# gradslam/gradslam

Hardware: NVIDIA H100
Metric: PointFusion frames/sec (640x480, B=8) (higher is better)
Workload: dtype f32

## Files before the change

gradslam_b200/_C.py:

```python
import ctypes
import os

import torch

_HERE = os.path.dirname(os.path.abspath(__file__))
LIB_PATH = os.environ.get("GSX_LIB_PATH") or os.path.join(_HERE, "_lib", "libgsx.so")

c_f32p = ctypes.c_void_p
c_i32p = ctypes.c_void_p
c_i64 = ctypes.c_int64
c_int = ctypes.c_int
c_float = ctypes.c_float
c_double = ctypes.c_double
c_u32 = ctypes.c_uint32
c_vp = ctypes.c_void_p

SIGNATURES = {
    "gsx_version": (c_int, []),
    "gsx_last_error": (ctypes.c_char_p, []),
    "gsx_backproject_normals_fwd": (
        c_int, [c_vp, c_i64, c_vp, c_i64, c_vp, c_i64, c_int, c_int, c_int, c_int, c_vp, c_vp, c_vp, c_vp, c_vp]),
    "gsx_backproject_normals_bwd_scratch_bytes": (c_i64, [c_int, c_int, c_int, c_int]),
    "gsx_backproject_normals_bwd": (
        c_int, [c_vp, c_i64, c_vp, c_i64, c_vp, c_i64, c_int, c_int, c_int, c_int, c_vp, c_vp, c_vp, c_vp, c_vp, c_vp,
                c_vp, c_i64, c_vp]),
    "gsx_fusion_workspace_bytes": (c_i64, [c_int, c_int, c_int]),
    "gsx_fusion_workspace_stats_offset": (c_i64, [c_int, c_int, c_int]),
    "gsx_fusion_frame_records": (
        c_int, [c_vp, c_i64, c_vp, c_i64, c_vp, c_i64, c_vp, c_vp, c_vp, c_int, c_int, c_int, c_double, c_vp, c_vp]),
    "gsx_fusion_project_select": (
        c_int, [c_vp, c_vp, c_i64, c_i64, c_vp, c_i64, c_vp, c_i64, c_int, c_int, c_int, c_float, c_float, c_vp, c_vp]),
    "gsx_fusion_merge_append": (
        c_int, [c_vp, c_vp, c_int, c_vp, c_vp, c_i64, c_vp, c_i64, c_int, c_int, c_int, c_vp, c_vp, c_vp, c_vp]),
    "gsx_fusion_merge_append_bwd": (
        c_int, [c_vp, c_vp, c_vp, c_vp, c_int, c_i64, c_vp, c_vp, c_i64, c_vp, c_vp, c_vp, c_vp, c_int, c_int, c_int,
                c_double, c_vp, c_vp, c_vp, c_vp, c_vp, c_vp, c_vp]),
    "gsx_pointfusion_sequence_groups": (c_int, [c_int]),
    "gsx_pointfusion_sequence_workspace_bytes": (c_i64, [c_int, c_int, c_int]),
    "gsx_pointfusion_sequence_gt": (
        c_int, [c_vp, c_vp, c_vp, c_i64, c_i64, c_vp, c_vp, c_vp, c_vp, c_int, c_int, c_int, c_int, c_int, c_int,
                c_float, c_float, c_double, c_vp, c_vp, c_vp]),
    "gsx_fusion_prune_scratch_bytes": (c_i64, [c_int, c_i64]),
    "gsx_fusion_prune_unstable": (
        c_int, [c_vp, c_vp, c_vp, c_i64, c_vp, c_int, c_int, c_int, c_float, c_int, c_vp, c_vp, c_i64, c_vp]),
    "gsx_fusion_prune_unstable_bwd": (c_int, [c_vp, c_vp, c_i64, c_vp, c_vp, c_i64, c_int, c_vp, c_vp, c_vp]),
    "gsx_pointfusion_sequence_gt_prune": (
        c_int, [c_vp, c_vp, c_vp, c_i64, c_i64, c_vp, c_vp, c_vp, c_vp, c_int, c_int, c_int, c_int, c_int, c_int,
                c_float, c_float, c_double, c_vp, c_vp, c_int, c_float, c_vp, c_i64, c_vp, c_vp]),
    "gsx_debug_fail_at_frame": (None, [c_int]),
    "gsx_debug_set_k2_grid_cap": (None, [c_int]),
    "gsx_peer_export": (c_int, [c_vp, c_vp, c_vp, c_vp]),
    "gsx_peer_open": (c_int, [c_vp, c_i64, c_vp]),
    "gsx_peer_close_all": (c_int, []),
    "gsx_peer_copy_rows": (c_int, [c_vp, c_i64, c_vp, c_i64, c_i64, c_i64, c_vp]),
    "gsx_ingest_raw": (c_int, [c_vp, c_vp, c_i64, c_double, c_int, c_vp, c_vp, c_vp]),
    "gsx_ingest_calibration": (c_int, [c_vp, c_i64, c_int, c_double, c_double, c_vp, c_vp, c_int, c_int, c_vp, c_vp,
                                       c_vp]),
    "gsx_compact_scratch_bytes": (c_i64, [c_i64]),
    "gsx_compact_indices": (c_int, [c_vp, c_i64, c_vp, c_vp, c_vp, c_u32, c_vp]),
    "gsx_active_eval": (c_int, [c_vp, c_vp, c_i64, c_i64, c_vp, c_i64, c_vp, c_i64, c_int, c_int, c_int, c_vp, c_vp,
                                c_vp]),
    "gsx_similar_eval": (c_int, [c_vp, c_i64, c_vp, c_i64, c_vp, c_vp, c_int, c_int, c_int, c_float, c_float, c_vp,
                                 c_vp]),
    "gsx_unique_select": (c_int, [c_vp, c_i64, c_vp, c_i64, c_vp, c_int, c_int, c_int, c_vp, c_vp, c_vp, c_vp]),
    "gsx_records_from_table": (c_int, [c_vp, c_i64, c_i64, c_int, c_int, c_int, c_vp, c_vp]),
    "gsx_knn1_scratch_bytes": (c_i64, [c_int, c_int, c_int]),
    "gsx_icp_tgt_scratch_bytes": (c_i64, [c_int, c_i64]),
    "gsx_knn1": (c_int, [c_vp, c_vp, c_int, c_vp, c_vp, c_int, c_int, c_vp, c_vp, c_vp, c_i64, c_int, c_vp]),
    "gsx_icp_normal_eq_scratch_bytes": (c_i64, [c_int]),
    "gsx_icp_normal_eq_fwd": (c_int, [c_vp, c_int, c_vp, c_vp, c_vp, c_vp, c_vp, c_i64, c_vp]),
    "gsx_icp_normal_eq_bwd": (c_int, [c_vp, c_int, c_vp, c_vp, c_vp, c_vp, c_vp, c_vp, c_vp, c_vp]),
    "gsx_icp_normal_eq_batched_fwd": (c_int, [c_vp, c_vp, c_int, c_vp, c_vp, c_int, c_int, c_vp, c_vp, c_vp, c_i64, c_vp]),
    "gsx_icp_normal_eq_batched_bwd": (c_int, [c_vp, c_vp, c_int, c_vp, c_vp, c_int, c_int, c_vp, c_vp, c_vp, c_vp, c_vp,
                                              c_vp]),
    "gsx_icp_solve_fwd": (c_int, [c_vp, c_vp, c_int, c_vp, c_vp, c_vp]),
    "gsx_icp_solve_bwd": (c_int, [c_vp, c_vp, c_int, c_vp, c_vp, c_vp, c_vp, c_vp]),
    "gsx_icp_update_fwd": (c_int, [c_vp, c_vp, c_vp, c_vp, c_vp, c_int, c_int, c_float, c_float, c_float, c_float,
                                   c_vp, c_vp, c_vp, c_vp]),
    "gsx_icp_update_bwd": (c_int, [c_vp, c_vp, c_vp, c_vp, c_vp, c_int, c_int, c_float, c_float, c_float, c_float,
                                   c_vp, c_vp, c_vp, c_vp, c_vp, c_vp, c_vp, c_vp, c_vp]),
    "gsx_rigid_transform_fwd": (c_int, [c_vp, c_i64, c_vp, c_vp, c_vp]),
    "gsx_rigid_transform_bwd_scratch_bytes": (c_i64, [c_i64]),
    "gsx_rigid_transform_batched_fwd": (c_int, [c_vp, c_vp, c_i64, c_int, c_vp, c_vp, c_vp]),
    "gsx_rigid_transform_batched_bwd": (c_int, [c_vp, c_vp, c_i64, c_int, c_vp, c_vp, c_vp, c_vp, c_vp, c_i64, c_vp]),
    "gsx_rigid_transform_bwd": (c_int, [c_vp, c_i64, c_vp, c_vp, c_vp, c_vp, c_vp, c_i64, c_vp]),
    "gsx_icp_align_scratch_bytes": (c_i64, [c_int, c_int, c_int]),
    "gsx_icp_align": (
        c_int, [c_vp, c_vp, c_int, c_vp, c_vp, c_vp, c_int, c_int, c_vp, c_int, c_int, c_float, c_int, c_float,
                c_float, c_float, c_float, c_float, c_vp, c_vp, c_vp, c_i64, c_vp]),
    "gsx_icp_workspace_bytes": (c_i64, [c_int, c_int, c_int, c_int, c_i64]),
    "gsx_icp_localize": (
        c_int, [c_vp, c_vp, c_i64, c_i64, c_vp, c_i64, c_vp, c_i64, c_vp, c_i64, c_int, c_int, c_int, c_int,
                c_int, c_int, c_float, c_int, c_float, c_float, c_float, c_float, c_float, c_vp, c_i64, c_vp, c_i64,
                c_vp, c_i64, c_u32, c_vp, c_vp]),
    "gsx_icp_projective_workspace_bytes": (c_i64, [c_int, c_int, c_int, c_int]),
    "gsx_icp_localize_projective": (
        c_int, [c_vp, c_vp, c_i64, c_i64, c_vp, c_i64, c_vp, c_i64, c_vp, c_i64, c_int, c_int, c_int, c_int, c_int,
                c_int, c_float, c_int, c_float, c_float, c_float, c_float, c_float, c_vp, c_i64, c_vp, c_i64, c_vp]),
    "gsx_icp_project_associate": (
        c_int, [c_vp, c_vp, c_int, c_vp, c_vp, c_vp, c_i64, c_vp, c_i64, c_int, c_int, c_int, c_int, c_float, c_vp, c_vp,
                c_vp]),
    "gsx_render_views": (
        c_int, [c_vp, c_vp, c_vp, c_i64, c_i64, c_vp, c_i64, c_vp, c_i64, c_int, c_int, c_int, c_int, c_vp, c_vp, c_vp,
                c_vp, c_vp, c_vp]),
    "gsx_render_views_bwd_scratch_bytes": (c_i64, [c_int, c_int, c_int, c_int]),
    "gsx_render_views_bwd": (
        c_int, [c_vp, c_vp, c_i64, c_vp, c_i64, c_vp, c_i64, c_vp, c_int, c_int, c_int, c_int, c_vp, c_vp, c_vp, c_vp,
                c_vp, c_vp, c_vp, c_vp, c_i64, c_vp]),
}

_lib = None


def lib():
    global _lib
    if _lib is None:
        if not os.path.exists(LIB_PATH):
            raise RuntimeError(
                "gradslam_b200: CUDA extension %s is missing. Build it with `python __graft_entry__.py build`. "
                "There is no CPU fallback." % LIB_PATH
            )
        handle = ctypes.CDLL(LIB_PATH)
        for name, (res, args) in SIGNATURES.items():
            fn = getattr(handle, name)
            fn.restype = res
            fn.argtypes = args
        _lib = handle
    return _lib


def check(rc, what):
    if rc != 0:
        raise RuntimeError("%s failed (status %d): %s" % (what, rc, lib().gsx_last_error().decode()))
# ... 45 lines not shown
```

gradslam_b200/csrc/gsx_fusion.cu:

```cuda
#include "gsx_common.cuh"
#include "gsx_exp.cuh"
#include "gsx_fusion_ws.cuh"
#include "gsx_thresholds.h"
#include "../../include/gsx.h"

namespace gsx {

constexpr int kBlock = 256;

__device__ __forceinline__ float confidence_exp(float sq_norm, float two_sigma_sq) {
  const float x = (-sq_norm) / two_sigma_sq;
  if (!(x >= -17.0f)) return 0.0f;
  return exp_f32_via_f64(x);
}
__device__ __forceinline__ float confidence_alpha(float sq_norm, float two_sigma_sq) {
  return fminf(fmaxf(confidence_exp(sq_norm, two_sigma_sq), 1e-7f), 1.01f);
}

struct FrameRecArgs {
  const float *depth;
  int64_t depth_bstride;
  const float *K;
  int64_t K_bstride;
  const float *poses;
  int64_t pose_bstride;
  const float *gv, *gn, *vloc;
  int B, H, W;
  float two_sigma_sq;
  Workspace ws;
};

constexpr int kRecTW = 32, kRecTH = 8;

__device__ __forceinline__ void store_frame_header(const FrameRecArgs &a, int b) {
  FrameHeader hd = {};
  hd.from_maps = a.gv != nullptr;
  if (!hd.from_maps) {
    hd.cam.k = load_kinv(a.K + b * a.K_bstride);
    if (a.poses) hd.cam.pose = load_rigid(a.poses + b * a.pose_bstride);
    hd.cam.posed = a.poses != nullptr;
  }
  hd.two_sigma_sq = a.two_sigma_sq;
  hd.depth = a.depth + b * a.depth_bstride;
  a.ws.hdr[b] = hd;
}

template <bool kAlpha>
__device__ __forceinline__ void frame_values(const FrameHeader &hd, bool from_maps, const Rigid *pose,
                                             const float4 *nrec, const float4 *vrec, int h, int w, int H, int W, float dc,
                                             float3 &gn, float4 &fv) {
  if (from_maps) {
    const float4 n = __ldg(nrec + h * W + w);
    gn = make_float3(n.x, n.y, n.z);
    fv = __ldg(vrec + h * W + w);
    return;
  }
  const FrameSample f = frame_sample_from(load_stencil_around(hd.depth, dc, h, w, H, W), hd.cam.k, pose, h, w, H, W);
  gn = f.gn;
  fv = make_float4(f.gv.x, f.gv.y, f.gv.z,
                   kAlpha ? confidence_alpha((f.v.x * f.v.x + f.v.y * f.v.y) + f.v.z * f.v.z, hd.two_sigma_sq) : 0.0f);
}

__device__ __forceinline__ float frame_depth(const FrameHeader &hd, bool from_maps, const float4 *nrec, int pix) {
  return from_maps ? __ldg(nrec + pix).w : __ldg(hd.depth + pix);
}

__device__ __forceinline__ void load_frame_header(FrameHeader &s, const FrameHeader *g) {
  constexpr int kWords = (int)(sizeof(FrameHeader) / 4);
  const int i = (int)threadIdx.x - 64;
  if (i >= 0 && i < kWords) reinterpret_cast<int *>(&s)[i] = __ldg(reinterpret_cast<const int *>(g) + i);
}

template <bool kFromMaps>
__global__ void __launch_bounds__(kRecTW *kRecTH) k_frame_records(FrameRecArgs a) {
  const int b = blockIdx.z;
  const int tid = threadIdx.y * kRecTW + threadIdx.x;
  const int lin = (blockIdx.y * gridDim.x + blockIdx.x) * (kRecTW * kRecTH) + tid;
  if (lin < a.ws.tiles) a.ws.tile_state[(int64_t)b * a.ws.tiles + lin] = 0ull;
  if (lin == 0) {
    a.ws.ticket[b] = 0u;
    store_frame_header(a, b);
  }
  const int w = blockIdx.x * kRecTW + threadIdx.x, h = blockIdx.y * kRecTH + threadIdx.y;
  if (w >= a.W || h >= a.H) return;
  const int P = a.H * a.W;
  const int pix = h * a.W + w;
  const int64_t i = (int64_t)b * P + pix;
  if (kFromMaps) {
    const int64_t o = i * 3;
    const float vx = __ldg(a.vloc + o), vy = __ldg(a.vloc + o + 1), vz = __ldg(a.vloc + o + 2);
    a.ws.nrec[i] = make_float4(__ldg(a.gn + o), __ldg(a.gn + o + 1), __ldg(a.gn + o + 2),
                               __ldg(a.depth + b * a.depth_bstride + pix));
    a.ws.vrec[i] = make_float4(__ldg(a.gv + o), __ldg(a.gv + o + 1), __ldg(a.gv + o + 2),
                               confidence_alpha((vx * vx + vy * vy) + vz * vz, a.two_sigma_sq));
  }
  a.ws.win[i] = 0u;
}

int launch_frame_records(const FrameRecArgs &a, cudaStream_t stream) {
  if (a.B == 0) return 0;
  const dim3 grid((unsigned)((a.W + kRecTW - 1) / kRecTW), (unsigned)((a.H + kRecTH - 1) / kRecTH), (unsigned)a.B);
  const dim3 block(kRecTW, kRecTH);
  if (a.gv)
    k_frame_records<true><<<grid, block, 0, stream>>>(a);
  else
    k_frame_records<false><<<grid, block, 0, stream>>>(a);
  GSX_CHECK_LAUNCH("gsx_fusion_frame_records");
  return 0;
}

struct ProjectArgs {
  const float *geo;
  const int32_t *counts;
  int64_t cap;
  const float *poses;
  int64_t pose_bstride;
  const float *K;
  int64_t K_bstride;
  int B;
  ImageBounds ib;
  float dot_th;
  float d2_max;
  const float4 *nrec, *vrec;
  const FrameHeader *hdr;
  unsigned int *win;
  unsigned long long *stats;
};

#ifndef GSX_K2_MINB
#define GSX_K2_MINB 4
#endif

struct MapRow {
  float4 a, b;
};
__device__ __forceinline__ MapRow load_map_row(const float *geo, int64_t n) {
  MapRow m;
  m.a = __ldg(reinterpret_cast<const float4 *>(geo + n * kGeoW));
  m.b = __ldg(reinterpret_cast<const float4 *>(geo + n * kGeoW + 4));
  return m;
}

template <bool kFromMaps>
__device__ __forceinline__ void select_rows(const ProjectArgs &a, const LiveCamera &s_cam, const FrameHeader &s_hdr,
                                            unsigned int *s_act, int b, int count) {
  const int P = a.ib.H * a.ib.W;
  const float *geo = a.geo + (int64_t)b * a.cap * kGeoW;
  const float4 *nrec = a.nrec + (int64_t)b * P, *vrec = a.vrec + (int64_t)b * P;
  unsigned int *win = a.win + (int64_t)b * P;
  const int64_t stride = (int64_t)gridDim.x * kBlock;
  int64_t n = (int64_t)blockIdx.x * kBlock + threadIdx.x;
  int pend_pix = -1;
  unsigned int pend_n = 0u, pend_old = 0u;
  unsigned long long pend_key = 0ull;
  float3 pend_fv = make_float3(0.f, 0.f, 0.f);
  MapRow cur = load_map_row(geo, n < count ? n : 0);
  for (; n < count; n += stride) {
    const MapRow m = cur;
    const int64_t nn = n + stride;
    if (nn < count) cur = load_map_row(geo, nn);
    const PixelHit hit = project(s_cam, a.ib, m.a.x, m.a.y, m.a.z);
    if (hit.in_frustum) {
      {
        const unsigned int am = __activemask();
        if ((int)(threadIdx.x & 31) == __ffs(am) - 1) atomicAdd(s_act + (threadIdx.x >> 5), (unsigned int)__popc(am));
      }
      const int pix = hit.h * a.ib.W + hit.w;
      float3 gn;
      float4 fv;
      frame_values<false>(s_hdr, kFromMaps, s_hdr.cam.posed ? &s_hdr.cam.pose : nullptr, nrec, vrec, hit.h, hit.w,
                          a.ib.H, a.ib.W, frame_depth(s_hdr, kFromMaps, nrec, pix), gn, fv);
      const float dot = (gn.x * m.a.w + gn.y * m.b.x) + gn.z * m.b.y;
      const float3 fv3 = make_float3(fv.x, fv.y, fv.z);
      const float d2 = ray_d2(fv3, m.a.x, m.a.y, m.a.z);
      const bool live = (d2 <= a.d2_max) && (dot > a.dot_th);
      if (pend_pix >= 0) {
        argmin_settle(win + pend_pix, pend_n, pend_key, pend_fv, geo, pend_old);
        pend_pix = -1;
      }
      if (live) {
        pend_n = (unsigned int)n;
        pend_key = argmin_key_hi(m.b.z, d2);
        pend_fv = fv3;
        pend_old = argmin_claim(win + pix, pend_n);
        pend_pix = pix;
      }
    }
  }
  if (pend_pix >= 0) argmin_settle(win + pend_pix, pend_n, pend_key, pend_fv, geo, pend_old);
}

__global__ void __launch_bounds__(kBlock, GSX_K2_MINB) k_project_select(ProjectArgs a) {
  __shared__ LiveCamera s_cam;
  __shared__ FrameHeader s_hdr;
  __shared__ unsigned int s_act[kBlock / 32];
  const int b = blockIdx.y;
  const int count = a.counts[b];
  if ((int64_t)blockIdx.x * kBlock >= count) return;
  load_live_camera(s_cam, a.poses, a.pose_bstride, a.K, a.K_bstride, b);
  load_frame_header(s_hdr, a.hdr + b);
  if (threadIdx.x < kBlock / 32) s_act[threadIdx.x] = 0u;
  __syncthreads();
  if (s_hdr.from_maps)
    select_rows<true>(a, s_cam, s_hdr, s_act, b, count);
  else
    select_rows<false>(a, s_cam, s_hdr, s_act, b, count);
  __syncthreads();
  if (threadIdx.x == 0) {
    unsigned int t = 0;
#pragma unroll
    for (int i = 0; i < kBlock / 32; ++i) t += s_act[i];
    if (t) atomicAdd(a.stats + 2 * b, (unsigned long long)t);
  }
}

#ifndef GSX_K2_CTAS_PER_SM
#define GSX_K2_CTAS_PER_SM 24
#endif

static int g_k2_grid_cap = 0;

int launch_project_select(const ProjectArgs &a, int64_t max_count, cudaStream_t stream) {
  if (a.B == 0 || max_count <= 0) return 0;
  int64_t bx = (max_count + kBlock - 1) / kBlock;
  const int64_t cap_blocks = g_k2_grid_cap > 0 ? (int64_t)g_k2_grid_cap : (int64_t)kNumSMs * GSX_K2_CTAS_PER_SM;
  if (bx * a.B > cap_blocks) bx = (cap_blocks + a.B - 1) / a.B;
  if (bx < 1) bx = 1;
  k_project_select<<<dim3((unsigned)bx, (unsigned)a.B), kBlock, 0, stream>>>(a);
  GSX_CHECK_LAUNCH("gsx_fusion_project_select");
  return 0;
}

struct MergeArgs {
  float *geo, *col;
  int with_cc;
  const int32_t *counts_in;
  int32_t *counts_out;
  int64_t cap;
  const float *rgb;
  int64_t rgb_bstride;
  int B, H, W;
  Workspace ws;
  int32_t *overflow;
  int32_t *assoc;
};

constexpr unsigned int kMergeEpoch = 1u;

#ifndef GSX_K4_MINB
#define GSX_K4_MINB 4
#endif

__device__ __forceinline__ void prefetch_l2(const float *p) { asm volatile("prefetch.global.L2 [%0];" ::"l"(p)); }

template <bool kAssoc>
__global__ void __launch_bounds__(kMB, GSX_K4_MINB) k_merge_append(MergeArgs a) {
  __shared__ int s_tile;
  __shared__ int s_warp_sums[kPix][kMB / 32];
  __shared__ int s_matched[kMB / 32];
  __shared__ int s_excl;
  __shared__ __align__(16) float s_rgb[kTilePix * 3];
  __shared__ FrameHeader s_hdr;
  const int b = blockIdx.x % a.B;
  const int T = a.ws.tiles;
  if (threadIdx.x == 0) s_tile = (int)atomicAdd(a.ws.ticket + b, 1u);
  load_frame_header(s_hdr, a.ws.hdr + b);
  const int count_in = a.counts_in[b];
  __syncthreads();
  const int tile = s_tile;
  const int P = a.H * a.W;
  const int lane = threadIdx.x & 31, warp = threadIdx.x >> 5;
  const int pix0 = tile * kTilePix;
  const unsigned int *win = a.ws.win + (int64_t)b * P;
  const float4 *nrec = a.ws.nrec + (int64_t)b * P, *vrec = a.ws.vrec + (int64_t)b * P;
  const float *rgb = a.rgb + b * a.rgb_bstride + (int64_t)pix0 * 3;

  const int tile_px = min(kTilePix, P - pix0);
  if ((reinterpret_cast<uintptr_t>(rgb) & 15) == 0) {
    const int n4 = (tile_px * 3) >> 2;
    for (int i = threadIdx.x; i < n4; i += kMB)
      reinterpret_cast<float4 *>(s_rgb)[i] = __ldg(reinterpret_cast<const float4 *>(rgb) + i);
    for (int i = (n4 << 2) + threadIdx.x; i < tile_px * 3; i += kMB) s_rgb[i] = __ldg(rgb + i);
  } else {
    for (int i = threadIdx.x; i < tile_px * 3; i += kMB) s_rgb[i] = __ldg(rgb + i);
  }

  int pix[kPix];
  unsigned int slot[kPix];
  float dep[kPix];
  bool matched[kPix], is_new[kPix];
#pragma unroll
  for (int j = 0; j < kPix; ++j) {
    pix[j] = pix0 + j * kMB + threadIdx.x;
    slot[j] = 0u;
    dep[j] = 0.0f;
    if (pix[j] < P) {
      slot[j] = win[pix[j]];
      dep[j] = frame_depth(s_hdr, s_hdr.from_maps, nrec, pix[j]);
    }
    matched[j] = a.with_cc && slot[j] != 0u;
    if (matched[j]) {
      const int64_t n = (int64_t)slot[j] - 1;
      prefetch_l2(a.geo + ((int64_t)b * a.cap + n) * kGeoW);
      prefetch_l2(a.col + ((int64_t)b * a.cap + n) * kColW);
    }
  }
  int n_matched = 0;
#pragma unroll
  for (int j = 0; j < kPix; ++j) n_matched += matched[j] ? 1 : 0;
  n_matched = __reduce_add_sync(0xffffffffu, n_matched);
  if (lane == 0) s_matched[warp] = n_matched;
  int new_off[kPix];
  const int block_total = block_offsets<kMB, kPix>(
      [&](int j) {
        is_new[j] = (pix[j] < P) && (dep[j] > 0.0f) && !matched[j];
        return is_new[j];
      },
      new_off, s_warp_sums,
      [&] {
        if (threadIdx.x == 0) {
          int t = 0;
#pragma unroll
          for (int i = 0; i < kMB / 32; ++i) t += s_matched[i];
          if (t) atomicAdd(a.ws.stats + 2 * b + 1, (unsigned long long)t);
        }
      });
  unsigned long long *state = a.ws.tile_state + (int64_t)b * T;
  if (threadIdx.x == 0) publish_tile(state, tile, T, kMergeEpoch, kTileAggregate, (unsigned)block_total);

  float *geo = a.geo + (int64_t)b * a.cap * kGeoW;
  float *col = a.col + (int64_t)b * a.cap * kColW;

  float4 fv[kPix];
  float3 fn[kPix];
#pragma unroll
  for (int j = 0; j < kPix; ++j) {
    if (matched[j] || is_new[j]) {
      const int ph = pix[j] / a.W;
      frame_values<true>(s_hdr, s_hdr.from_maps, s_hdr.cam.posed ? &s_hdr.cam.pose : nullptr, nrec, vrec, ph, pix[j] - ph * a.W, a.H, a.W, dep[j], fn[j], fv[j]);
    }
  }

  float4 g0[kPix], g1[kPix], c4[kPix];
#pragma unroll
  for (int j = 0; j < kPix; ++j) {
    if (matched[j]) {
      const int64_t n = (int64_t)slot[j] - 1;
      g0[j] = *reinterpret_cast<const float4 *>(geo + n * kGeoW);
      g1[j] = *reinterpret_cast<const float4 *>(geo + n * kGeoW + 4);
      c4[j] = *reinterpret_cast<const float4 *>(col + n * kColW);
    }
  }
#pragma unroll
  for (int j = 0; j < kPix; ++j) {
    if (matched[j]) {
      const int64_t n = (int64_t)slot[j] - 1;
      const float alpha = fv[j].w;
      const float c0 = g1[j].z;
      const float tot = c0 + alpha;
      const float inv = 1.0f / ((tot == 0.0f) ? 1.0f : tot);
      const float *fc = s_rgb + (j * kMB + (int)threadIdx.x) * 3;
      float4 o0, o1, oc;
      o0.x = ((c0 * g0[j].x) + (alpha * fv[j].x)) * inv;
      o0.y = ((c0 * g0[j].y) + (alpha * fv[j].y)) * inv;
      o0.z = ((c0 * g0[j].z) + (alpha * fv[j].z)) * inv;
      o0.w = ((c0 * g0[j].w) + (alpha * fn[j].x)) * inv;
      o1.x = ((c0 * g1[j].x) + (alpha * fn[j].y)) * inv;
      o1.y = ((c0 * g1[j].y) + (alpha * fn[j].z)) * inv;
      o1.z = tot;
      o1.w = 0.0f;
      oc.x = ((c0 * c4[j].x) + (alpha * fc[0])) * inv;
      oc.y = ((c0 * c4[j].y) + (alpha * fc[1])) * inv;
      oc.z = ((c0 * c4[j].z) + (alpha * fc[2])) * inv;
      oc.w = 0.0f;
      *reinterpret_cast<float4 *>(geo + n * kGeoW) = o0;
      *reinterpret_cast<float4 *>(geo + n * kGeoW + 4) = o1;
      *reinterpret_cast<float4 *>(col + n * kColW) = oc;
      if (kAssoc) a.assoc[(int64_t)b * P + pix[j]] = -(int32_t)(n + 1);
    }
  }

  if (warp == 0) {
    const unsigned int excl = lookback_warp(state, tile, T, kMergeEpoch, (unsigned)block_total);
    if (lane == 0) s_excl = (int)excl;
  }
  __syncthreads();
  const int64_t base = (int64_t)count_in + s_excl;
#pragma unroll
  for (int j = 0; j < kPix; ++j) {
    if (is_new[j]) {
      const int64_t n = base + new_off[j];
      if (n < a.cap) {
        const float *fc = s_rgb + (j * kMB + (int)threadIdx.x) * 3;
        *reinterpret_cast<float4 *>(geo + n * kGeoW) = make_float4(fv[j].x, fv[j].y, fv[j].z, fn[j].x);
        *reinterpret_cast<float4 *>(geo + n * kGeoW + 4) =
            make_float4(fn[j].y, fn[j].z, a.with_cc ? fv[j].w : 0.0f, 0.0f);
        *reinterpret_cast<float4 *>(col + n * kColW) = make_float4(fc[0], fc[1], fc[2], 0.0f);
        if (kAssoc) a.assoc[(int64_t)b * P + pix[j]] = (int32_t)(n + 1);
      } else {
        *a.overflow = 1;
      }
    }
  }
  if (tile == T - 1 && threadIdx.x == 0) {
    const int64_t total = base + block_total;
    a.counts_out[b] = (int32_t)(total < a.cap ? total : a.cap);
  }
}

int launch_merge_append(const MergeArgs &a, cudaStream_t stream) {
  if (a.B == 0) return 0;
  const dim3 grid((unsigned)(a.ws.tiles * a.B));
  if (a.assoc)
    k_merge_append<true><<<grid, kMB, 0, stream>>>(a);
  else
    k_merge_append<false><<<grid, kMB, 0, stream>>>(a);
  GSX_CHECK_LAUNCH("gsx_fusion_merge_append");
  return 0;
}

struct MergeBwdArgs {
  const int32_t *assoc;
  const int32_t *counts_in;
  const float *geo, *col;
  int with_cc;
  int64_t cap_in;
  const float *g_geo, *g_col;
  int64_t cap_out;
  const float *gv, *gn, *rgb, *vloc;
  float *d_geo, *d_col;
  float *d_gv, *d_gn, *d_rgb, *d_vloc;
  int B, P;
  float two_sigma_sq;
};

__global__ void __launch_bounds__(256) k_merge_bwd_rows(MergeBwdArgs a) {
  const int b = blockIdx.y;
  const int64_t n = (int64_t)blockIdx.x * blockDim.x + threadIdx.x;
  if (n >= a.cap_in) return;
  const bool live = n < a.counts_in[b] && n < a.cap_out;
  const int64_t ri = (int64_t)b * a.cap_in + n, ro = (int64_t)b * a.cap_out + n;
  float4 z = make_float4(0.f, 0.f, 0.f, 0.f), g0 = z, g1 = z, gc = z;
  if (live && a.g_geo) {
    g0 = *reinterpret_cast<const float4 *>(a.g_geo + ro * kGeoW);
    g1 = *reinterpret_cast<const float4 *>(a.g_geo + ro * kGeoW + 4);
    g1.w = 0.0f;
    if (!a.with_cc) g1.z = 0.0f;
  }
  if (live && a.g_col) {
    gc = *reinterpret_cast<const float4 *>(a.g_col + ro * kColW);
    gc.w = 0.0f;
  }
  *reinterpret_cast<float4 *>(a.d_geo + ri * kGeoW) = g0;
  *reinterpret_cast<float4 *>(a.d_geo + ri * kGeoW + 4) = g1;
  *reinterpret_cast<float4 *>(a.d_col + ri * kColW) = gc;
}

__global__ void __launch_bounds__(256) k_merge_bwd_pixels(MergeBwdArgs a) {
  const int b = blockIdx.y;
  const int pix = blockIdx.x * blockDim.x + threadIdx.x;
  if (pix >= a.P) return;
  const int64_t fi = ((int64_t)b * a.P + pix) * 3;
  const int32_t as = a.assoc[(int64_t)b * a.P + pix];
  float dgv[3] = {0.f, 0.f, 0.f}, dgn[3] = {0.f, 0.f, 0.f}, dc[3] = {0.f, 0.f, 0.f}, dv[3] = {0.f, 0.f, 0.f};
  if (as != 0) {
    const int64_t n = (as > 0) ? (int64_t)as - 1 : -(int64_t)as - 1;
    const int64_t ro = (int64_t)b * a.cap_out + n;
    float g[9];
#pragma unroll
    for (int q = 0; q < 6; ++q) g[q] = a.g_geo ? a.g_geo[ro * kGeoW + q] : 0.0f;
#pragma unroll
    for (int q = 0; q < 3; ++q) g[6 + q] = a.g_col ? a.g_col[ro * kColW + q] : 0.0f;
    const float gcc = (a.g_geo && a.with_cc) ? a.g_geo[ro * kGeoW + 6] : 0.0f;
    const float vx = a.vloc[fi], vy = a.vloc[fi + 1], vz = a.vloc[fi + 2];
    const float sq = (vx * vx + vy * vy) + vz * vz;
    const float e = (float)exp((double)((-sq) / a.two_sigma_sq));
    float d_alpha = gcc;
    if (as > 0) {
#pragma unroll
      for (int q = 0; q < 3; ++q) {
        dgv[q] = g[q];
        dgn[q] = g[3 + q];
        dc[q] = g[6 + q];
      }
    } else {
      const int64_t ri = (int64_t)b * a.cap_in + n;
      const float alpha = fminf(fmaxf(e, 1e-7f), 1.01f);
      const float c0 = a.geo[ri * kGeoW + 6];
      const float tot = c0 + alpha;
      const bool degenerate = tot == 0.0f;
      const float inv = 1.0f / (degenerate ? 1.0f : tot);
      const float dinv = degenerate ? 0.0f : -(inv * inv);
      float f[9], m[9];
#pragma unroll
      for (int q = 0; q < 3; ++q) {
        f[q] = a.gv[fi + q];
        f[3 + q] = a.gn[fi + q];
        f[6 + q] = a.rgb[fi + q];
        m[q] = a.geo[ri * kGeoW + q];
        m[3 + q] = a.geo[ri * kGeoW + 3 + q];
        m[6 + q] = a.col[ri * kColW + q];
      }
      float d_c0 = gcc;
      float dm[9], df[9];
#pragma unroll
      for (int q = 0; q < 9; ++q) {
        const float num = c0 * m[q] + alpha * f[q];
        dm[q] = g[q] * c0 * inv;
        df[q] = g[q] * alpha * inv;
        d_c0 += g[q] * (m[q] * inv + num * dinv);
        d_alpha += g[q] * (f[q] * inv + num * dinv);
      }
#pragma unroll
      for (int q = 0; q < 6; ++q) a.d_geo[ri * kGeoW + q] = dm[q];
      a.d_geo[ri * kGeoW + 6] = d_c0;
#pragma unroll
      for (int q = 0; q < 3; ++q) {
        a.d_col[ri * kColW + q] = dm[6 + q];
        dgv[q] = df[q];
        dgn[q] = df[3 + q];
        dc[q] = df[6 + q];
      }
    }
    if (e >= 1e-7f && e <= 1.01f) {
      const float s = d_alpha * e * (-2.0f / a.two_sigma_sq);
      dv[0] = s * vx;
      dv[1] = s * vy;
      dv[2] = s * vz;
    }
  }
#pragma unroll
  for (int q = 0; q < 3; ++q) {
    a.d_gv[fi + q] = dgv[q];
    a.d_gn[fi + q] = dgn[q];
    a.d_rgb[fi + q] = dc[q];
    a.d_vloc[fi + q] = dv[q];
  }
}

static Workspace group_workspace(void *workspace, int B_total, int b0, int H, int W) {
  const int64_t P = (int64_t)H * W;
  Workspace ws = fusion_workspace(workspace, B_total, H, W);
  ws.nrec += (int64_t)b0 * P;
  ws.vrec += (int64_t)b0 * P;
  ws.hdr += b0;
  ws.win += (int64_t)b0 * P;
  ws.tile_state += (int64_t)b0 * ws.tiles;
  ws.ticket += b0;
  ws.stats += 2 * b0;
  return ws;
}

int fusion_records_group(const float *poses, int64_t pose_bs, const float *K, int64_t K_bs, const float *depth,
                         int64_t d_bs, int B_total, int b0, int nb, int H, int W, double sigma, void *workspace,
                         cudaStream_t st) {
  FrameRecArgs fa{depth + (int64_t)b0 * d_bs, d_bs, K + (int64_t)b0 * K_bs, K_bs, poses + (int64_t)b0 * pose_bs, pose_bs,
                  nullptr, nullptr, nullptr, nb, H, W, (float)(2.0 * (sigma * sigma)),
                  group_workspace(workspace, B_total, b0, H, W)};
  return launch_frame_records(fa, st);
}

int fusion_update_group(float *geo, float *col, const int32_t *cin, int32_t *cout, int64_t cap, int64_t max_count,
                        const float *poses, int64_t pose_bs, const float *K, int64_t K_bs, const float *rgb,
                        int64_t rgb_bs, int B_total, int b0, int nb, int H, int W, float dist_th, float dot_th,
                        void *workspace, int32_t *overflow, cudaStream_t st) {
  const Workspace ws = group_workspace(workspace, B_total, b0, H, W);
  float *ggeo = geo + (int64_t)b0 * cap * kGeoW, *gcol = col + (int64_t)b0 * cap * kColW;
  if (max_count > 0) {
    ProjectArgs pa{ggeo, cin + b0, cap, poses + (int64_t)b0 * pose_bs, pose_bs, K + (int64_t)b0 * K_bs, K_bs, nb,
                   image_bounds(H, W), dot_th, sqrt_lt_threshold(dist_th), ws.nrec, ws.vrec, ws.hdr, ws.win, ws.stats};
    const int rc = launch_project_select(pa, max_count, st);
    if (rc) return rc;
  }
  MergeArgs ma{ggeo, gcol, 1, cin + b0, cout + b0, cap, rgb + (int64_t)b0 * rgb_bs, rgb_bs, nb, H, W, ws, overflow, nullptr};
  return launch_merge_append(ma, st);
}

int64_t fusion_workspace_bytes(int B, int H, int W) {
  int64_t bytes;
  fusion_workspace(nullptr, B, H, W, &bytes);
  return bytes;
}

}

using namespace gsx;

extern "C" int64_t gsx_fusion_workspace_bytes(int B, int H, int W) {
  if (B < 0 || H < 0 || W < 0) return -1;
  return fusion_workspace_bytes(B, H, W);
}

extern "C" int64_t gsx_fusion_workspace_stats_offset(int B, int H, int W) {
  if (B < 0 || H < 0 || W < 0) return -1;
  return (int64_t)reinterpret_cast<uintptr_t>(fusion_workspace(nullptr, B, H, W).stats);
}

static bool aligned16(const void *p) { return (reinterpret_cast<uintptr_t>(p) & 15) == 0; }

extern "C" int gsx_fusion_frame_records(const float *depth, int64_t depth_bstride, const float *intrinsics,
                                        int64_t K_bstride, const float *poses, int64_t pose_bstride,
                                        const float *gvertex, const float *gnormal, const float *vertex, int B, int H,
                                        int W, double sigma, void *workspace, void *stream) {
  GSX_CHECK_ARG(B >= 0 && H >= 2 && W >= 2, "gsx_fusion_frame_records: bad extents B=%d H=%d W=%d", B, H, W);
  if (B == 0) return 0;
  GSX_CHECK_ARG(depth && workspace, "gsx_fusion_frame_records: null pointer");
  GSX_CHECK_ARG((gvertex && gnormal && vertex) || (!gvertex && !gnormal && !vertex && intrinsics),
                "gsx_fusion_frame_records: pass the three frame maps, or none of them together with the intrinsics");
  GSX_CHECK_ARG(aligned16(workspace), "gsx_fusion_frame_records: the workspace must be 16-byte aligned");
  FrameRecArgs a{depth, depth_bstride, intrinsics, K_bstride, poses, pose_bstride, gvertex, gnormal, vertex, B, H, W,
                 (float)(2.0 * (sigma * sigma)), fusion_workspace(workspace, B, H, W)};
  return launch_frame_records(a, (cudaStream_t)stream);
}

extern "C" int gsx_fusion_project_select(const float *map_geometry, const int32_t *counts, int64_t capacity,
                                         int64_t max_count, const float *poses, int64_t pose_bstride,
                                         const float *intrinsics, int64_t K_bstride, int B, int H, int W,
                                         float dist_th, float dot_th, void *workspace, void *stream) {
  GSX_CHECK_ARG(B >= 0 && H >= 2 && W >= 2, "gsx_fusion_project_select: bad extents B=%d H=%d W=%d", B, H, W);
  if (max_count <= 0 || B == 0) return 0;
  GSX_CHECK_ARG(map_geometry && counts, "gsx_fusion_project_select: null map pointer");
  GSX_CHECK_ARG(poses && intrinsics && workspace, "gsx_fusion_project_select: null frame pointer");
  GSX_CHECK_ARG(aligned16(map_geometry) && aligned16(workspace),
                "gsx_fusion_project_select: geometry rows and workspace must be 16-byte aligned");
  GSX_CHECK_ARG(max_count <= capacity, "gsx_fusion_project_select: max_count %lld > capacity %lld",
                (long long)max_count, (long long)capacity);
  const Workspace ws = fusion_workspace(workspace, B, H, W);
  ProjectArgs a{map_geometry, counts, capacity, poses, pose_bstride, intrinsics, K_bstride, B, image_bounds(H, W),
                dot_th, sqrt_lt_threshold(dist_th), ws.nrec, ws.vrec, ws.hdr, ws.win, ws.stats};
  return launch_project_select(a, max_count, (cudaStream_t)stream);
}

extern "C" void gsx_debug_set_k2_grid_cap(int ctas) { g_k2_grid_cap = ctas > 0 ? ctas : 0; }

extern "C" int gsx_fusion_merge_append(float *map_geometry, float *map_colors, int with_ccounts,
                                       const int32_t *counts_in, int32_t *counts_out, int64_t capacity,
                                       const float *rgb, int64_t rgb_bstride, int B, int H, int W, void *workspace,
                                       int32_t *overflow_flag, int32_t *assoc_out, void *stream) {
  GSX_CHECK_ARG(B >= 0 && H >= 2 && W >= 2, "gsx_fusion_merge_append: bad extents B=%d H=%d W=%d", B, H, W);
  if (B == 0) return 0;
  GSX_CHECK_ARG(map_geometry && map_colors && counts_in && counts_out, "gsx_fusion_merge_append: null map pointer");
  GSX_CHECK_ARG(counts_in != counts_out, "gsx_fusion_merge_append: counts_in and counts_out must not alias");
  GSX_CHECK_ARG(rgb && workspace && overflow_flag, "gsx_fusion_merge_append: null frame pointer");
  GSX_CHECK_ARG(aligned16(map_geometry) && aligned16(map_colors) && aligned16(workspace),
                "gsx_fusion_merge_append: map rows and workspace must be 16-byte aligned");
  GSX_CHECK_ARG(capacity <= 0x7fffffffll, "gsx_fusion_merge_append: capacity must fit int32 (counts are int32)");
  MergeArgs a{map_geometry, map_colors, with_ccounts ? 1 : 0, counts_in, counts_out, capacity, rgb, rgb_bstride, B, H,
              W, fusion_workspace(workspace, B, H, W), overflow_flag, assoc_out};
  return launch_merge_append(a, (cudaStream_t)stream);
}

extern "C" int gsx_fusion_merge_append_bwd(const int32_t *assoc, const int32_t *counts_in, const float *map_geometry,
                                           const float *map_colors, int with_ccounts, int64_t capacity_in,
                                           const float *g_geometry, const float *g_colors, int64_t capacity_out,
                                           const float *gvertex, const float *gnormal, const float *rgb,
                                           const float *vertex, int B, int H, int W, double sigma,
                                           float *d_map_geometry, float *d_map_colors, float *d_gvertex,
                                           float *d_gnormal, float *d_rgb, float *d_vertex, void *stream) {
  GSX_CHECK_ARG(B >= 0 && H >= 2 && W >= 2, "gsx_fusion_merge_append_bwd: bad extents B=%d H=%d W=%d", B, H, W);
  if (B == 0) return 0;
  GSX_CHECK_ARG(assoc && counts_in && gvertex && gnormal && rgb && vertex, "gsx_fusion_merge_append_bwd: null input");
  GSX_CHECK_ARG(d_gvertex && d_gnormal && d_rgb && d_vertex, "gsx_fusion_merge_append_bwd: null frame gradient");
  GSX_CHECK_ARG(capacity_in == 0 || (map_geometry && map_colors && d_map_geometry && d_map_colors),
                "gsx_fusion_merge_append_bwd: null map pointer");
  GSX_CHECK_ARG(aligned16(map_geometry) && aligned16(map_colors) && aligned16(g_geometry) && aligned16(g_colors) &&
                    aligned16(d_map_geometry) && aligned16(d_map_colors),
                "gsx_fusion_merge_append_bwd: map rows must be 16-byte aligned");
  MergeBwdArgs a{assoc, counts_in, map_geometry, map_colors, with_ccounts ? 1 : 0, capacity_in, g_geometry, g_colors,
                 capacity_out, gvertex, gnormal, rgb, vertex, d_map_geometry, d_map_colors, d_gvertex, d_gnormal, d_rgb,
                 d_vertex, B, H * W, (float)(2.0 * (sigma * sigma))};
  cudaStream_t st = (cudaStream_t)stream;
  if (capacity_in > 0) {
    k_merge_bwd_rows<<<dim3((unsigned)((capacity_in + 255) / 256), (unsigned)B), 256, 0, st>>>(a);
    GSX_CHECK_LAUNCH("gsx_fusion_merge_append_bwd(rows)");
  }
  k_merge_bwd_pixels<<<dim3((unsigned)((a.P + 255) / 256), (unsigned)B), 256, 0, st>>>(a);
  GSX_CHECK_LAUNCH("gsx_fusion_merge_append_bwd(pixels)");
  return 0;
}
```

gradslam_b200/csrc/gsx_fusion_ws.cuh:

```cuda
#pragma once
#include "gsx_common.cuh"

namespace gsx {

#ifndef GSX_KPIX
#define GSX_KPIX 2
#endif
constexpr int kMB = 256;
constexpr int kPix = GSX_KPIX;
constexpr int kTilePix = kMB * kPix;

struct FrameHeader {
  FrameCamera cam;
  float two_sigma_sq;
  int from_maps;
  const float *depth;
};

struct Workspace {
  float4 *nrec, *vrec;
  FrameHeader *hdr;
  unsigned int *win;
  unsigned long long *tile_state;
  unsigned int *ticket;
  unsigned long long *stats;
  int tiles;
};

inline Workspace fusion_workspace(void *base, int B, int H, int W, int64_t *bytes = nullptr) {
  const int64_t P = (int64_t)H * W;
  Carver c(base);
  Workspace w;
  w.tiles = (int)((P + kTilePix - 1) / kTilePix);
  w.nrec = c.take<float4>(B * P);
  w.vrec = c.take<float4>(B * P);
  w.hdr = c.take<FrameHeader>(B);
  w.win = c.take<unsigned int>(B * P);
  w.tile_state = c.take<unsigned long long>((int64_t)B * w.tiles);
  w.ticket = c.take<unsigned int>(B);
  w.stats = c.take<unsigned long long>(2 * (int64_t)B);
  if (bytes) *bytes = c.bytes;
  return w;
}

}
```

include/gsx.h:

```cpp
#ifndef GSX_H_
#define GSX_H_

#include <stdint.h>

#ifdef __cplusplus
extern "C" {
#endif

#define GSX_VERSION 200

int gsx_version(void);
const char *gsx_last_error(void);

int gsx_backproject_normals_fwd(const float *depth, int64_t depth_bstride, const float *intrinsics,
                                int64_t K_bstride, const float *poses, int64_t pose_bstride, int B, int L,
                                int H, int W, float *vertex, float *normal, float *gvertex, float *gnormal,
                                void *stream);

int64_t gsx_backproject_normals_bwd_scratch_bytes(int B, int L, int H, int W);
int gsx_backproject_normals_bwd(const float *depth, int64_t depth_bstride, const float *intrinsics,
                                int64_t K_bstride, const float *poses, int64_t pose_bstride, int B, int L,
                                int H, int W, const float *g_vertex, const float *g_normal,
                                const float *g_gvertex, const float *g_gnormal, float *g_depth,
                                float *g_poses, void *scratch, int64_t scratch_bytes, void *stream);

int64_t gsx_fusion_workspace_bytes(int B, int H, int W);
int64_t gsx_fusion_workspace_stats_offset(int B, int H, int W);

int gsx_fusion_frame_records(const float *depth, int64_t depth_bstride, const float *intrinsics, int64_t K_bstride,
                             const float *poses, int64_t pose_bstride, const float *gvertex, const float *gnormal,
                             const float *vertex, int B, int H, int W, double sigma, void *workspace, void *stream);

int gsx_fusion_project_select(const float *map_geometry, const int32_t *counts, int64_t capacity, int64_t max_count,
                              const float *poses, int64_t pose_bstride, const float *intrinsics, int64_t K_bstride,
                              int B, int H, int W, float dist_th, float dot_th, void *workspace, void *stream);

int gsx_fusion_merge_append(float *map_geometry, float *map_colors, int with_ccounts, const int32_t *counts_in,
                            int32_t *counts_out, int64_t capacity, const float *rgb, int64_t rgb_bstride, int B, int H,
                            int W, void *workspace, int32_t *overflow_flag, int32_t *assoc_out, void *stream);

int gsx_fusion_merge_append_bwd(const int32_t *assoc, const int32_t *counts_in, const float *map_geometry,
                                const float *map_colors, int with_ccounts, int64_t capacity_in,
                                const float *g_geometry, const float *g_colors, int64_t capacity_out,
                                const float *gvertex, const float *gnormal, const float *rgb, const float *vertex,
                                int B, int H, int W, double sigma, float *d_map_geometry, float *d_map_colors,
                                float *d_gvertex, float *d_gnormal, float *d_rgb, float *d_vertex, void *stream);

int gsx_pointfusion_sequence_groups(int B);
int64_t gsx_pointfusion_sequence_workspace_bytes(int B, int H, int W);
int gsx_pointfusion_sequence_gt(float *map_geometry, float *map_colors, int32_t *counts, int64_t capacity,
                                int64_t max_count0, const float *depth, const float *rgb, const float *intrinsics,
                                const float *poses, int B, int L, int s_begin, int s_end, int H, int W, float dist_th,
                                float dot_th, double sigma, void *workspace, int32_t *overflow_flag, void *stream);
int64_t gsx_fusion_prune_scratch_bytes(int B, int64_t capacity);
int gsx_fusion_prune_unstable(float *map_geometry, float *map_colors, int32_t *counts, int64_t capacity, int32_t *ring,
                              int ring_len, int step, int t_max, float c_stable, int B, int32_t *keep_map,
                              void *scratch, int64_t scratch_bytes, void *stream);
int gsx_fusion_prune_unstable_bwd(const int32_t *keep_map, const int32_t *counts_in, int64_t capacity_in,
                                  const float *g_geometry, const float *g_colors, int64_t capacity_out, int B,
                                  float *d_map_geometry, float *d_map_colors, void *stream);
int gsx_pointfusion_sequence_gt_prune(float *map_geometry, float *map_colors, int32_t *counts, int64_t capacity,
                                      int64_t max_count0, const float *depth, const float *rgb, const float *intrinsics,
                                      const float *poses, int B, int L, int s_begin, int s_end, int H, int W,
                                      float dist_th, float dot_th, double sigma, void *workspace, int32_t *ring,
                                      int t_max, float c_stable, void *prune_scratch, int64_t prune_scratch_bytes,
                                      int32_t *overflow_flag, void *stream);
void gsx_debug_fail_at_frame(int s);
void gsx_debug_set_k2_grid_cap(int ctas);

#define GSX_IPC_HANDLE_BYTES 64
int gsx_peer_export(const void *ptr, unsigned char *handle , int64_t *offset,
                    int64_t *allocation_bytes );
int gsx_peer_open(const unsigned char *handle, int64_t offset, void **ptr_out);
int gsx_peer_close_all(void);
int gsx_peer_copy_rows(void *dst, int64_t dst_pitch_bytes, const void *src, int64_t src_pitch_bytes,
                       int64_t width_bytes, int64_t n_blocks, void *stream);

int gsx_ingest_raw(const uint8_t *rgb_u8, const uint16_t *depth_u16, int64_t n_pixels, double depth_scaling_factor,
                   int normalize_color, float *rgb_out, float *depth_out, void *stream);

int gsx_ingest_calibration(const float *intrinsics, int64_t n_intrinsics, int intrinsics_dim, double h_ratio,
                           double w_ratio, float *intrinsics_out, const float *poses, int B, int L, float *poses_out,
                           int32_t *singular_flag, void *stream);


int64_t gsx_compact_scratch_bytes(int64_t n);
int gsx_compact_indices(const uint8_t *flags, int64_t n, int64_t *out_idx, int64_t *out_count, void *scratch,
                        uint32_t epoch, void *stream);

int gsx_active_eval(const float *map_geometry, const int32_t *counts, int64_t capacity, int64_t width,
                    const float *poses, int64_t pose_bstride, const float *intrinsics, int64_t K_bstride, int B,
                    int H, int W, uint8_t *flags, int32_t *hw, void *stream);

int gsx_similar_eval(const int64_t *table, int64_t rows, const float *map_geometry, int64_t capacity,
                     const float *gvertex, const float *gnormal, int B, int H, int W, float dist_th, float dot_th,
                     uint8_t *flags, void *stream);

int gsx_unique_select(const int64_t *table, int64_t rows, const float *map_geometry, int64_t capacity,
                      const float *gvertex, int B, int H, int W, void *records, uint8_t *pixel_flags,
                      int64_t *pixel_n, void *stream);

int gsx_records_from_table(const int64_t *table, int64_t rows, int64_t capacity, int B, int H, int W,
                           void *workspace, void *stream);


int64_t gsx_knn1_scratch_bytes(int B, int ns_stride, int nt_stride);
int gsx_knn1(const float *src_points, const int32_t *src_count, int ns_stride, const float *tgt_points,
             const int32_t *tgt_count, int nt_stride, int B, int64_t *idx_out, float *d2_out, void *scratch,
             int64_t scratch_bytes, int build_grid, void *stream);

int64_t gsx_icp_normal_eq_scratch_bytes(int ns);
int gsx_icp_normal_eq_fwd(const float *src_points, int ns, const float *tgt_points, const float *tgt_normals,
                          const int64_t *nn_idx, float *sums_out, void *scratch, int64_t scratch_bytes, void *stream);
int gsx_icp_normal_eq_bwd(const float *src_points, int ns, const float *tgt_points, const float *tgt_normals,
                          const int64_t *nn_idx, const float *g_sums, float *g_src, float *g_tgt_points_rows,
                          float *g_tgt_normals_rows, void *stream);

int gsx_icp_normal_eq_batched_fwd(const float *src_points, const int32_t *src_count, int ns_stride,
                                  const float *tgt_points, const float *tgt_normals, int nt_stride, int B,
                                  const int64_t *nn_idx, float *sums_out, void *scratch, int64_t scratch_bytes,
                                  void *stream);
int gsx_icp_normal_eq_batched_bwd(const float *src_points, const int32_t *src_count, int ns_stride,
                                  const float *tgt_points, const float *tgt_normals, int nt_stride, int B,
                                  const int64_t *nn_idx, const float *g_sums, float *g_src, float *g_tgt_points_rows,
                                  float *g_tgt_normals_rows, void *stream);
int gsx_icp_solve_fwd(const float *sums, const float *damp, int n, float *xi_out, float *dT_out, void *stream);
int gsx_icp_solve_bwd(const float *sums, const float *damp, int n, const float *g_xi, const float *g_dT,
                      float *g_sums, float *g_damp, void *stream);
int gsx_icp_update_fwd(const float *xi, const float *err, const float *new_err, const float *damp, const float *T,
                       int n, int mode, float lambda_max, float B, float B2, float nu, float *damp_out,
                       float *dT_out, float *T_out, void *stream);
int gsx_icp_update_bwd(const float *xi, const float *err, const float *new_err, const float *damp, const float *T,
                       int n, int mode, float lambda_max, float B, float B2, float nu, const float *g_damp_out,
                       const float *g_dT_out, const float *g_T_out, float *g_xi, float *g_err, float *g_new_err,
                       float *g_damp, float *g_T, void *stream);

int gsx_rigid_transform_fwd(const float *points, int64_t n, const float *T, float *out, void *stream);
int64_t gsx_rigid_transform_bwd_scratch_bytes(int64_t n);
int gsx_rigid_transform_batched_fwd(const float *points, const int32_t *counts, int64_t stride, int B, const float *T,
                                    float *out, void *stream);
int gsx_rigid_transform_batched_bwd(const float *points, const int32_t *counts, int64_t stride, int B, const float *T,
                                    const float *g_out, float *g_points, float *g_T, void *scratch,
                                    int64_t scratch_bytes, void *stream);
int gsx_rigid_transform_bwd(const float *points, int64_t n, const float *T, const float *g_out, float *g_points,
                            float *g_T, void *scratch, int64_t scratch_bytes, void *stream);

int64_t gsx_icp_align_scratch_bytes(int B, int ns_stride, int nt_stride);
int gsx_icp_align(const float *src_points, const int32_t *src_count, int ns_stride, const float *tgt_points,
                  const float *tgt_normals, const int32_t *tgt_count, int nt_stride, int B,
                  const float *initial_transform, int mode, int numiters, float damp, int use_dist_thresh,
                  float dist_thresh, float lambda_max, float Bp, float B2p, float nu, float *transform_out,
// ... 41 lines not shown
```

Before: 27440.

## Bin projection candidates per tile and resolve argmin in merge shared memory

```diff
diff --git a/gradslam_b200/_C.py b/gradslam_b200/_C.py
--- a/gradslam_b200/_C.py
+++ b/gradslam_b200/_C.py
@@ -49,6 +49,7 @@
                 c_float, c_float, c_double, c_vp, c_vp, c_int, c_float, c_vp, c_i64, c_vp, c_vp]),
     "gsx_debug_fail_at_frame": (None, [c_int]),
     "gsx_debug_set_k2_grid_cap": (None, [c_int]),
+    "gsx_debug_set_bin_capacity": (None, [c_int]),
     "gsx_peer_export": (c_int, [c_vp, c_vp, c_vp, c_vp]),
     "gsx_peer_open": (c_int, [c_vp, c_i64, c_vp]),
     "gsx_peer_close_all": (c_int, []),
diff --git a/gradslam_b200/csrc/gsx_fusion.cu b/gradslam_b200/csrc/gsx_fusion.cu
--- a/gradslam_b200/csrc/gsx_fusion.cu
+++ b/gradslam_b200/csrc/gsx_fusion.cu
@@ -76,7 +76,10 @@
   const int b = blockIdx.z;
   const int tid = threadIdx.y * kRecTW + threadIdx.x;
   const int lin = (blockIdx.y * gridDim.x + blockIdx.x) * (kRecTW * kRecTH) + tid;
-  if (lin < a.ws.tiles) a.ws.tile_state[(int64_t)b * a.ws.tiles + lin] = 0ull;
+  if (lin < a.ws.tiles) {
+    a.ws.tile_state[(int64_t)b * a.ws.tiles + lin] = 0ull;
+    a.ws.bin_count[(int64_t)b * a.ws.tiles + lin] = 0u;
+  }
   if (lin == 0) {
     a.ws.ticket[b] = 0u;
     store_frame_header(a, b);
@@ -125,10 +128,14 @@
   const FrameHeader *hdr;
   unsigned int *win;
   unsigned long long *stats;
+  unsigned int *bin_count;
+  uint4 *bin;
+  int tiles;
+  int bin_cap;
 };
 
 #ifndef GSX_K2_MINB
-#define GSX_K2_MINB 4
+#define GSX_K2_MINB 5
 #endif
 
 struct MapRow {
@@ -141,6 +148,22 @@
   return m;
 }
 
+__device__ __forceinline__ void append_candidate(unsigned int *bin_count, uint4 *bin, int bin_cap, unsigned int *win,
+                                                 const float *geo, int pix, unsigned int n,
+                                                 unsigned long long key_hi, const float3 &fv) {
+  const int t = pix / kTilePix;
+  const unsigned int grp = __match_any_sync(__activemask(), t);
+  const int lane = (int)(threadIdx.x & 31), leader = __ffs(grp) - 1;
+  unsigned int base = 0u;
+  if (lane == leader) base = atomicAdd(bin_count + t, (unsigned int)__popc(grp));
+  const unsigned int s = __shfl_sync(grp, base, leader) + (unsigned int)__popc(grp & ((1u << lane) - 1u));
+  if (s < (unsigned int)bin_cap)
+    bin[(int64_t)t * kBinCap + s] =
+        make_uint4((unsigned int)key_hi, (unsigned int)(key_hi >> 32), n, (unsigned int)(pix - t * kTilePix));
+  else
+    argmin_settle(win + pix, n, key_hi, fv, geo, argmin_claim(win + pix, n));
+}
+
 template <bool kFromMaps>
 __device__ __forceinline__ void select_rows(const ProjectArgs &a, const LiveCamera &s_cam, const FrameHeader &s_hdr,
                                             unsigned int *s_act, int b, int count) {
@@ -148,12 +171,10 @@
   const float *geo = a.geo + (int64_t)b * a.cap * kGeoW;
   const float4 *nrec = a.nrec + (int64_t)b * P, *vrec = a.vrec + (int64_t)b * P;
   unsigned int *win = a.win + (int64_t)b * P;
+  unsigned int *bin_count = a.bin_count + (int64_t)b * a.tiles;
+  uint4 *bin = a.bin + (int64_t)b * a.tiles * kBinCap;
   const int64_t stride = (int64_t)gridDim.x * kBlock;
   int64_t n = (int64_t)blockIdx.x * kBlock + threadIdx.x;
-  int pend_pix = -1;
-  unsigned int pend_n = 0u, pend_old = 0u;
-  unsigned long long pend_key = 0ull;
-  float3 pend_fv = make_float3(0.f, 0.f, 0.f);
   MapRow cur = load_map_row(geo, n < count ? n : 0);
   for (; n < count; n += stride) {
     const MapRow m = cur;
@@ -174,20 +195,10 @@
       const float3 fv3 = make_float3(fv.x, fv.y, fv.z);
       const float d2 = ray_d2(fv3, m.a.x, m.a.y, m.a.z);
       const bool live = (d2 <= a.d2_max) && (dot > a.dot_th);
-      if (pend_pix >= 0) {
-        argmin_settle(win + pend_pix, pend_n, pend_key, pend_fv, geo, pend_old);
-        pend_pix = -1;
-      }
-      if (live) {
-        pend_n = (unsigned int)n;
-        pend_key = argmin_key_hi(m.b.z, d2);
-        pend_fv = fv3;
-        pend_old = argmin_claim(win + pix, pend_n);
-        pend_pix = pix;
-      }
-    }
-  }
-  if (pend_pix >= 0) argmin_settle(win + pend_pix, pend_n, pend_key, pend_fv, geo, pend_old);
+      if (live)
+        append_candidate(bin_count, bin, a.bin_cap, win, geo, pix, (unsigned int)n, argmin_key_hi(m.b.z, d2), fv3);
+    }
+  }
 }
 
 __global__ void __launch_bounds__(kBlock, GSX_K2_MINB) k_project_select(ProjectArgs a) {
@@ -220,8 +231,13 @@
 
 static int g_k2_grid_cap = 0;
 
-int launch_project_select(const ProjectArgs &a, int64_t max_count, cudaStream_t stream) {
-  if (a.B == 0 || max_count <= 0) return 0;
+static int g_bin_cap = -1;
+static int bin_capacity() { return g_bin_cap >= 0 && g_bin_cap < kBinCap ? g_bin_cap : kBinCap; }
+
+int launch_project_select(const ProjectArgs &args, int64_t max_count, cudaStream_t stream) {
+  if (args.B == 0 || max_count <= 0) return 0;
+  ProjectArgs a = args;
+  a.bin_cap = bin_capacity();
   int64_t bx = (max_count + kBlock - 1) / kBlock;
   const int64_t cap_blocks = g_k2_grid_cap > 0 ? (int64_t)g_k2_grid_cap : (int64_t)kNumSMs * GSX_K2_CTAS_PER_SM;
   if (bx * a.B > cap_blocks) bx = (cap_blocks + a.B - 1) / a.B;
@@ -243,6 +259,7 @@
   Workspace ws;
   int32_t *overflow;
   int32_t *assoc;
+  int bin_cap;
 };
 
 constexpr unsigned int kMergeEpoch = 1u;
@@ -261,9 +278,15 @@
   __shared__ int s_excl;
   __shared__ __align__(16) float s_rgb[kTilePix * 3];
   __shared__ FrameHeader s_hdr;
+  __shared__ unsigned long long s_key[kTilePix];
+  __shared__ unsigned int s_n[kTilePix];
   const int b = blockIdx.x % a.B;
   const int T = a.ws.tiles;
   if (threadIdx.x == 0) s_tile = (int)atomicAdd(a.ws.ticket + b, 1u);
+  for (int i = threadIdx.x; i < kTilePix; i += kMB) {
+    s_key[i] = ~0ull;
+    s_n[i] = ~0u;
+  }
   load_frame_header(s_hdr, a.ws.hdr + b);
   const int count_in = a.counts_in[b];
   __syncthreads();
@@ -274,6 +297,8 @@
   const unsigned int *win = a.ws.win + (int64_t)b * P;
   const float4 *nrec = a.ws.nrec + (int64_t)b * P, *vrec = a.ws.vrec + (int64_t)b * P;
   const float *rgb = a.rgb + b * a.rgb_bstride + (int64_t)pix0 * 3;
+  const int n_bin = (int)min(a.ws.bin_count[(int64_t)b * T + tile], (unsigned int)a.bin_cap);
+  const uint4 *bin = a.ws.bin + ((int64_t)b * T + tile) * kBinCap;
 
   const int tile_px = min(kTilePix, P - pix0);
   if ((reinterpret_cast<uintptr_t>(rgb) & 15) == 0) {
@@ -297,6 +322,47 @@
     if (pix[j] < P) {
       slot[j] = win[pix[j]];
       dep[j] = frame_depth(s_hdr, s_hdr.from_maps, nrec, pix[j]);
+    }
+  }
+
+  static_assert(kBinCap % kMB == 0, "a bin is read in whole rounds of the CTA");
+  constexpr int kRec = kBinCap / kMB;
+  uint4 rec[kRec];
+#pragma unroll
+  for (int k = 0; k < kRec; ++k) {
+    const int i = k * kMB + (int)threadIdx.x;
+    if (i < n_bin) rec[k] = __ldg(bin + i);
+  }
+#pragma unroll
+  for (int k = 0; k < kRec; ++k)
+    if (k * kMB + (int)threadIdx.x < n_bin) atomicMin(s_key + rec[k].w, ((unsigned long long)rec[k].y << 32) | rec[k].x);
+  __syncthreads();
+#pragma unroll
+  for (int k = 0; k < kRec; ++k)
+    if (k * kMB + (int)threadIdx.x < n_bin &&
+        (((unsigned long long)rec[k].y << 32) | rec[k].x) == s_key[rec[k].w])
+      atomicMin(s_n + rec[k].w, rec[k].z);
+  __syncthreads();
+
+#pragma unroll
+  for (int j = 0; j < kPix; ++j) {
+    const int q = j * kMB + (int)threadIdx.x;
+    const unsigned int bn = s_n[q];
+    if (bn != ~0u) {
+      if (slot[j] == 0u) {
+        slot[j] = bn + 1u;
+      } else {
+        const int ph = pix[j] / a.W;
+        float3 gn;
+        float4 fv;
+        frame_values<false>(s_hdr, s_hdr.from_maps, s_hdr.cam.posed ? &s_hdr.cam.pose : nullptr, nrec, vrec, ph,
+                            pix[j] - ph * a.W, a.H, a.W, dep[j], gn, fv);
+        const unsigned int m = slot[j] - 1u;
+        const float4 p = *reinterpret_cast<const float4 *>(a.geo + ((int64_t)b * a.cap + m) * kGeoW);
+        const unsigned long long k = argmin_key_hi(a.geo[((int64_t)b * a.cap + m) * kGeoW + 6],
+                                                   ray_d2(make_float3(fv.x, fv.y, fv.z), p.x, p.y, p.z));
+        if (!(k < s_key[q] || (k == s_key[q] && m < bn))) slot[j] = bn + 1u;
+      }
     }
     matched[j] = a.with_cc && slot[j] != 0u;
     if (matched[j]) {
@@ -408,8 +474,10 @@
   }
 }
 
-int launch_merge_append(const MergeArgs &a, cudaStream_t stream) {
-  if (a.B == 0) return 0;
+int launch_merge_append(const MergeArgs &args, cudaStream_t stream) {
+  if (args.B == 0) return 0;
+  MergeArgs a = args;
+  a.bin_cap = bin_capacity();
   const dim3 grid((unsigned)(a.ws.tiles * a.B));
   if (a.assoc)
     k_merge_append<true><<<grid, kMB, 0, stream>>>(a);
@@ -546,6 +614,8 @@
   ws.hdr += b0;
   ws.win += (int64_t)b0 * P;
   ws.tile_state += (int64_t)b0 * ws.tiles;
+  ws.bin_count += (int64_t)b0 * ws.tiles;
+  ws.bin += (int64_t)b0 * ws.tiles * kBinCap;
   ws.ticket += b0;
   ws.stats += 2 * b0;
   return ws;
@@ -568,11 +638,11 @@
   float *ggeo = geo + (int64_t)b0 * cap * kGeoW, *gcol = col + (int64_t)b0 * cap * kColW;
   if (max_count > 0) {
     ProjectArgs pa{ggeo, cin + b0, cap, poses + (int64_t)b0 * pose_bs, pose_bs, K + (int64_t)b0 * K_bs, K_bs, nb,
-                   image_bounds(H, W), dot_th, sqrt_lt_threshold(dist_th), ws.nrec, ws.vrec, ws.hdr, ws.win, ws.stats};
+                   image_bounds(H, W), dot_th, sqrt_lt_threshold(dist_th), ws.nrec, ws.vrec, ws.hdr, ws.win, ws.stats, ws.bin_count, ws.bin, ws.tiles, 0};
     const int rc = launch_project_select(pa, max_count, st);
     if (rc) return rc;
   }
-  MergeArgs ma{ggeo, gcol, 1, cin + b0, cout + b0, cap, rgb + (int64_t)b0 * rgb_bs, rgb_bs, nb, H, W, ws, overflow, nullptr};
+  MergeArgs ma{ggeo, gcol, 1, cin + b0, cout + b0, cap, rgb + (int64_t)b0 * rgb_bs, rgb_bs, nb, H, W, ws, overflow, nullptr, 0};
   return launch_merge_append(ma, st);
 }
 
@@ -627,11 +697,13 @@
                 (long long)max_count, (long long)capacity);
   const Workspace ws = fusion_workspace(workspace, B, H, W);
   ProjectArgs a{map_geometry, counts, capacity, poses, pose_bstride, intrinsics, K_bstride, B, image_bounds(H, W),
-                dot_th, sqrt_lt_threshold(dist_th), ws.nrec, ws.vrec, ws.hdr, ws.win, ws.stats};
+                dot_th, sqrt_lt_threshold(dist_th), ws.nrec, ws.vrec, ws.hdr, ws.win, ws.stats, ws.bin_count, ws.bin, ws.tiles, 0};
   return launch_project_select(a, max_count, (cudaStream_t)stream);
 }
 
 extern "C" void gsx_debug_set_k2_grid_cap(int ctas) { g_k2_grid_cap = ctas > 0 ? ctas : 0; }
+
+extern "C" void gsx_debug_set_bin_capacity(int records) { g_bin_cap = records >= 0 ? records : -1; }
 
 extern "C" int gsx_fusion_merge_append(float *map_geometry, float *map_colors, int with_ccounts,
                                        const int32_t *counts_in, int32_t *counts_out, int64_t capacity,
@@ -646,7 +718,7 @@
                 "gsx_fusion_merge_append: map rows and workspace must be 16-byte aligned");
   GSX_CHECK_ARG(capacity <= 0x7fffffffll, "gsx_fusion_merge_append: capacity must fit int32 (counts are int32)");
   MergeArgs a{map_geometry, map_colors, with_ccounts ? 1 : 0, counts_in, counts_out, capacity, rgb, rgb_bstride, B, H,
-              W, fusion_workspace(workspace, B, H, W), overflow_flag, assoc_out};
+              W, fusion_workspace(workspace, B, H, W), overflow_flag, assoc_out, 0};
   return launch_merge_append(a, (cudaStream_t)stream);
 }
 
diff --git a/gradslam_b200/csrc/gsx_fusion_ws.cuh b/gradslam_b200/csrc/gsx_fusion_ws.cuh
--- a/gradslam_b200/csrc/gsx_fusion_ws.cuh
+++ b/gradslam_b200/csrc/gsx_fusion_ws.cuh
@@ -9,6 +9,11 @@
 constexpr int kMB = 256;
 constexpr int kPix = GSX_KPIX;
 constexpr int kTilePix = kMB * kPix;
+
+#ifndef GSX_BIN_CAP
+#define GSX_BIN_CAP 1024
+#endif
+constexpr int kBinCap = GSX_BIN_CAP;
 
 struct FrameHeader {
   FrameCamera cam;
@@ -22,6 +27,8 @@
   FrameHeader *hdr;
   unsigned int *win;
   unsigned long long *tile_state;
+  unsigned int *bin_count;
+  uint4 *bin;
   unsigned int *ticket;
   unsigned long long *stats;
   int tiles;
@@ -37,6 +44,8 @@
   w.hdr = c.take<FrameHeader>(B);
   w.win = c.take<unsigned int>(B * P);
   w.tile_state = c.take<unsigned long long>((int64_t)B * w.tiles);
+  w.bin_count = c.take<unsigned int>((int64_t)B * w.tiles);
+  w.bin = c.take<uint4>((int64_t)B * w.tiles * kBinCap);
   w.ticket = c.take<unsigned int>(B);
   w.stats = c.take<unsigned long long>(2 * (int64_t)B);
   if (bytes) *bytes = c.bytes;
diff --git a/include/gsx.h b/include/gsx.h
--- a/include/gsx.h
+++ b/include/gsx.h
@@ -67,6 +67,7 @@
                                       int32_t *overflow_flag, void *stream);
 void gsx_debug_fail_at_frame(int s);
 void gsx_debug_set_k2_grid_cap(int ctas);
+void gsx_debug_set_bin_capacity(int records);
 
 #define GSX_IPC_HANDLE_BYTES 64
 int gsx_peer_export(const void *ptr, unsigned char *handle , int64_t *offset,
```

Measured after the change: 30160, median of 6. 1.1x the previous value.
